# afford-motion/afford-motion

Hardware: AMD Instinct MI355X
Metric: denoising steps/sec (B=32, L=196, N=8192) (higher is better)
Workload: dtype f32

## Files before the change

afford-motion_amd/afm/cmdm.py:

```python
from __future__ import annotations

import ctypes as C
import math
from typing import Dict, List, Optional

import torch
import torch.nn as nn

from . import autograd as AG
from . import ffi, ops
from ._cache import HeldKey
from .base import Model
from .scene import SceneMapEncoder, SceneMapEncoderDecoder
from .text import TextEncoderMixin, lang_feat_dim_type


def compute_repr_dimesion(data_repr: str) -> int:
    table = {"smplx_no_hands": 69, "pos": 66, "pos_rot": 129, "contact_one_joints": 1, "contact_all_joints": 22,
             "contact_cont_joints": 6, "contact_pelvis": 1, "h3d": 263}
    if data_repr not in table:
        raise ValueError(f"Unknown data representation: {data_repr}")
    return table[data_repr]


# ... 148 lines not shown
        self.all_queries = False
        self.no_ln_fold = False
        self.pair_launch = False
        self.fused_layernorm = False
        self._pack = None
        self._cond_cache = None
        self._ws: Dict[tuple, torch.Tensor] = {}

    def _weights(self) -> ffi.CmdmWeights:
        ver = (_param_version(self), self.training)
        if self._pack is not None and self._pack[0] == ver:
            return self._stamp(self._pack[1])
        dev = self.motion_adapter.weight.device
        if dev.type != "cuda":
            raise ffi.AfmError("CMDM parameters are on the CPU; move the model to the MI355X (`model.to('cuda')`)")
        keep: List[torch.Tensor] = []

        def P(t: torch.Tensor) -> int:
            t = ffi.f32c(t.detach())
            keep.append(t)
            return t.data_ptr()

        w = ffi.CmdmWeights()
        layers = self.self_attn_layer.layers
        w.d, w.heads, w.ff, w.n_layers = self.latent_dim, self.num_heads, layers[0].linear1.out_features, len(layers)
        w.motion_dim = self.motion_dim
        w.n_cond = 1 + self.contact_encoder.num_groups
        kpad = -(-self.motion_dim // 16) * 16
        w.motion_adapter_kpad = kpad if (kpad != self.motion_dim and kpad >= 128) else 0
        maw = self.motion_adapter.weight.detach()
        if w.motion_adapter_kpad:
            maw = torch.nn.functional.pad(maw, (0, kpad - self.motion_dim))
        w.motion_adapter_w, w.motion_adapter_b = P(maw), P(self.motion_adapter.bias)
        w.motion_layer_w, w.motion_layer_b = P(self.motion_layer.weight), P(self.motion_layer.bias)
        w.time_table, w.n_timesteps = P(self.timestep_embedder.table()), self.timestep_embedder.pe.shape[0]
        w.pos_table = P(self.positional_encoder.pe[:, 0, :])
        for i, l in enumerate(layers):
            lw = w.layer[i]
            lw.in_proj_w, lw.in_proj_b = P(l.self_attn.in_proj_weight), P(l.self_attn.in_proj_bias)
            lw.out_proj_w, lw.out_proj_b = P(l.self_attn.out_proj.weight), P(l.self_attn.out_proj.bias)
            lw.lin1_w, lw.lin1_b, lw.lin2_w, lw.lin2_b = P(l.linear1.weight), P(l.linear1.bias), P(l.linear2.weight), P(l.linear2.bias)
            lw.norm1_w, lw.norm1_b, lw.norm2_w, lw.norm2_b = P(l.norm1.weight), P(l.norm1.bias), P(l.norm2.weight), P(l.norm2.bias)
        if not self.training:
            import numpy as np

            def fold(lin_w, lin_b, norm):
                wd = lin_w.detach().cpu().numpy().astype(np.float64)
                gam, bet = norm.weight.detach().cpu().numpy().astype(np.float64), norm.bias.detach().cpu().numpy().astype(np.float64)
                wg = wd * gam[None, :]
                up = lambda a: torch.from_numpy(np.ascontiguousarray(a.astype(np.float32))).to(dev)
                return P(up(wg)), P(up(wg.sum(1))), P(up(lin_b.detach().cpu().numpy().astype(np.float64) + wd @ bet))
            for i, l in enumerate(layers):
                lw = w.layer[i]
                lw.lin1_wg, lw.lin1_g, lw.lin1_c = fold(l.linear1.weight, l.linear1.bias, l.norm1)
                if i > 0:
                    lw.in_proj_wg, lw.in_proj_g, lw.in_proj_c = fold(l.self_attn.in_proj_weight, l.self_attn.in_proj_bias, layers[i - 1].norm2)
            w.motion_layer_wg, w.motion_layer_g, w.motion_layer_c = fold(self.motion_layer.weight, self.motion_layer.bias, layers[-1].norm2)
        self._pack = (ver, w, keep)
        return self._stamp(w)

    def _stamp(self, w: ffi.CmdmWeights) -> ffi.CmdmWeights:
        w.gemm_arith, w.gemm_arith_min_n = ops.gemm_arith()
        w.attn_group_waves = int(self.attn_group_waves)
        w.flags = (ffi.CMDM_NO_L0_CACHE if self.no_l0_cache else 0) | (ffi.CMDM_FUSED_LN if self.fused_layernorm else 0) | \
            (ffi.CMDM_NO_LN_FOLD if self.no_ln_fold else 0) | (ffi.CMDM_ALL_QUERIES if self.all_queries else 0) | (ffi.CMDM_NO_RIDERS if self.no_riders else 0) | ((int(self.gemm_tile) & 0xF) << 8) | \
            (ffi.CMDM_PAIR_LAUNCH if self.pair_launch else 0)
        return w

    def _workspace(self, w: ffi.CmdmWeights, B: int, L: int, device) -> torch.Tensor:
        key = (B, L, str(device))
        if key not in self._ws:
            nbytes = ffi.load().afm_cmdm_workspace_bytes(C.byref(w), B, L)
            if nbytes < 0:
# ... 375 lines not shown
```

afford-motion_amd/afm/ffi.py:

```python
from __future__ import annotations

import ctypes as C
import os
from typing import Optional

import torch

_LIB_PATH = os.path.join(os.path.dirname(os.path.abspath(__file__)), "libafm_hip.so")
_lib = None

ACT_NONE, ACT_GELU, ACT_RELU, ACT_SILU = 0, 1, 2, 3
ARITH_DEFAULT, ARITH_F32, ARITH_BF16X1, ARITH_BF16X6, ARITH_BF16X9 = 0, 1, 3, 6, 9
TUNE_NO_DMA, TUNE_TILE_SHIFT = 0x1, 4
CMDM_NO_L0_CACHE, CMDM_FUSED_LN, CMDM_NO_LN_FOLD, CMDM_ALL_QUERIES, CMDM_CLIP_X0, CMDM_NO_RIDERS, CMDM_PAIR_LAUNCH = 0x1, 0x2, 0x4, 0x8, 0x10, 0x20, 0x40
CDM_NO_GEN, CDM_CHAIN_SIDE, CDM_DEC_CHUNKS_SHIFT, CDM_CLIP_X0, CDM_PIPELINE = 0x2, 0x4, 12, 0x8, 0x10
ABI_VERSION = 7
MAX_LAYERS = 16

c_f32p = C.c_void_p
i32, i64, u64 = C.c_int32, C.c_int64, C.c_uint64


class AfmError(RuntimeError):
    pass
# ... 119 lines not shown
                ("per_sample", i64), ("seed", u64), ("sample_index0", i64), ("step", i32)]


class ImputeStepArgs(C.Structure):
    _fields_ = [("x0_c", c_f32p), ("x0_u", c_f32p), ("scale", c_f32p), ("known", c_f32p), ("mask", C.c_void_p), ("x_t", c_f32p),
                ("noise", c_f32p), ("x_next", c_f32p), ("c1", c_f32p), ("c2", c_f32p), ("sigma", c_f32p), ("ddim", C.POINTER(DdimRows)),
                ("clip", i32), ("B", i32), ("per_sample", i64), ("seed", u64), ("sample_index0", i64), ("step", i32)]


CFG_FORCE_MASKED = 0x1

EXPORTS = {
    "afm_version": (C.c_int, []),
    "afm_linear": (C.c_int, [C.POINTER(LinearArgs), C.c_void_p]),
    "afm_linear_pair": (C.c_int, [C.POINTER(LinearArgs), C.POINTER(LinearArgs), C.c_void_p]),
    "afm_mha_fwd": (C.c_int, [c_f32p, C.c_void_p, c_f32p, i32, i32, i32, i32, C.c_void_p]),
    "afm_mha_fwd_grouped": (C.c_int, [c_f32p, C.c_void_p, c_f32p, i32, i32, i32, i32, i32, C.c_void_p]),
    "afm_clamp": (C.c_int, [c_f32p, i64, C.c_float, C.c_float, C.c_void_p]),
    "afm_mha_fwd_rows": (C.c_int, [c_f32p, C.c_void_p, c_f32p, i32, i32, i32, i32, i32, i32, C.c_void_p]),
    "afm_mha_fwd_arith": (C.c_int, [c_f32p, C.c_void_p, c_f32p, i32, i32, i32, i32, i32, i32, i32, C.c_void_p]),
    "afm_mha_cross_fwd": (C.c_int, [c_f32p, c_f32p, C.c_void_p, c_f32p, i32, i32, i32, i32, i32, C.c_void_p]),
    "afm_layernorm": (C.c_int, [c_f32p, c_f32p, c_f32p, c_f32p, i64, i32, C.c_float, C.c_void_p]),
    "afm_layernorm_rows": (C.c_int, [c_f32p, c_f32p, c_f32p, c_f32p, i64, i32, C.c_float, i32, i32, i32, C.c_void_p]),
    "afm_ddpm_step": (C.c_int, [c_f32p, c_f32p, c_f32p, c_f32p, c_f32p, c_f32p, c_f32p, i32, i64, u64, i64, i32, C.c_void_p]),
    "afm_randn": (C.c_int, [c_f32p, i32, i64, u64, i64, i32, C.c_void_p]),
    "afm_ddim_step": (C.c_int, [c_f32p, c_f32p, c_f32p, c_f32p, C.POINTER(DdimRows), i32, i64, u64, i64, i32, C.c_void_p]),
    "afm_ddim_sched_scratch_bytes": (i64, [i32, i32]),
    "afm_cmdm_ddim_loop_range": (C.c_int, [C.POINTER(CmdmWeights), c_f32p, c_f32p, C.c_void_p, c_f32p, C.c_void_p, C.POINTER(DdimRows),
                                           i32, i32, u64, i64, i32, i32, C.c_void_p, C.c_void_p, i64, i32, C.POINTER(C.c_void_p), C.c_void_p]),
    "afm_cdm_ddim_loop_range": (C.c_int, [C.POINTER(CdmWeights), c_f32p, c_f32p, c_f32p, c_f32p, c_f32p, c_f32p, C.c_void_p, C.POINTER(DdimRows),
# ... 179 lines not shown


def require_gpu(*tensors: torch.Tensor) -> None:
    for t in tensors:
        if t is not None and not t.is_cuda:
            raise AfmError("afford-motion_amd runs on the MI355X HIP path only; got a CPU tensor "
                           "(the CPU oracle lives in oracle/ and is test infrastructure)")


def f32c(t: torch.Tensor) -> torch.Tensor:
    if t.dtype != torch.float32:
        t = t.float()
    return t if t.is_contiguous() else t.contiguous()


def profile_enable(on: bool) -> None:
    check(load().afm_profile_enable(1 if on else 0), "afm_profile_enable")


def profile_read():
    buf = (ProfileEntry * 32)()
    n = load().afm_profile_read(buf, 32)
    if n < 0:
        check(n, "afm_profile_read")
    return {buf[i].name.decode(): dict(launches=buf[i].launches, total_ms=buf[i].total_ms, total_work=buf[i].total_work)
            for i in range(n)}


def progress_slices(n_steps: int, progress: bool, slices: int = 50):
    if not progress:
# ... 53 lines not shown
```

afford-motion_amd/csrc/cmdm.hip:

```cpp
#include <memory>

#include "sample_loop.h"

using namespace afm_loop;

extern "C" int afm_linear(const afm_linear_args*, void*);
extern "C" int afm_linear_pair(const afm_linear_args*, const afm_linear_args*, void*);
extern "C" int afm_mha_fwd_grouped(const float*, const uint8_t*, float*, int32_t, int32_t, int32_t, int32_t, int32_t, void*);
extern "C" int afm_mha_fwd_rows(const float*, const uint8_t*, float*, int32_t, int32_t, int32_t, int32_t, int32_t, int32_t, void*);
extern "C" int afm_mha_fwd_arith(const float*, const uint8_t*, float*, int32_t, int32_t, int32_t, int32_t, int32_t, int32_t, int32_t, void*);
extern "C" int afm_layernorm(const float*, const float*, const float*, float*, int64_t, int32_t, float, void*);
extern "C" int afm_layernorm_rows(const float*, const float*, const float*, float*, int64_t, int32_t, float, int32_t, int32_t, int32_t, void*);
extern "C" int afm_randn(float*, int32_t, int64_t, uint64_t, int64_t, int32_t, void*);

namespace {

struct Workspace {
    float *seq0, *y, *x1, *tmp, *qkv, *qkv0, *att, *hid, *noise, *xpad;
    float* x0;
    uint8_t* keymask;
    uint32_t* lncnt;
    float *stat1, *stat2;
    int64_t bytes;
};
// ... 409 lines not shown
        sb = {};
        sub_range(a.B, p->nsub, s, &sb.start, &sb.count);
        off += carve_sub(*c.w, c.cfg ? &p->wu : nullptr, c.L, (char*)a.workspace + off, &sb);
        sb.stream = p->nsub > 1 ? (hipStream_t)a.streams[s] : (hipStream_t)a.stream;
        if (p->branch_streams) sb.branch = (hipStream_t)c.cfg->branch_streams[s];
    }
    if (off > a.workspace_bytes) return AFM_E_WORKSPACE;

    const int T = 1 + c.w->n_cond + c.L;
    p->w = *c.w;
    p->w.flags = a.loop_flags(p->w.flags);
    if (c.cfg || c.mask) p->w.flags = (p->w.flags | AFM_PRIV_DDIM) & ~(AFM_CMDM_PAIR_LAUNCH | AFM_CMDM_FUSED_LN);
    if (p->nsub >= 2 && ((p->w.flags >> AFM_CMDM_WIDE_TILE_SHIFT) & 0xF) == 0) {
        bool big = true;
        for (int s = 0; s < p->nsub; ++s) big = big && (int64_t)p->sb[s].count * T >= 4096;
        if (big) p->w.flags |= 14 << AFM_CMDM_WIDE_TILE_SHIFT;
    }
    if (c.cfg) { const int nc_u = p->wu.n_cond; p->wu = p->w; p->wu.n_cond = nc_u; }
    p->paired = (p->w.flags & AFM_CMDM_PAIR_LAUNCH) && p->nsub == 2 && p->sb[0].count > 0 && p->sb[1].count > 0;
    p->row = (int64_t)c.L * c.w->motion_dim;
    return 0;
}

struct Loop {
    const LoopCall& c;
    LoopPlan p;
    Schedule sched;
};

inline float* sub_x(const Loop& l, const SubBatch& sb) { return l.c.x + (int64_t)sb.start * l.p.row; }

// ... 211 lines not shown
```

afford-motion_amd/csrc/gemm.hip:

```cpp
#include <type_traits>
#include "common.h"
#include "profile.h"
#include "gemm_epilogue.h"

namespace {

constexpr int BK = 32;
constexpr int LDK = 36;

template <int ROWS, bool VEC>
__device__ __forceinline__ void load_tile(const float* const (&rowp)[ROWS / 32], int k, int K, float4 (&reg)[ROWS / 32]) {
#pragma unroll
    for (int i = 0; i < ROWS / 32; ++i) {
        if (VEC) {
            reg[i] = *reinterpret_cast<const float4*>(rowp[i] + min(k, K - 4));
        } else {
            const float* p = rowp[i];
            reg[i] = make_float4(p[min(k, K - 1)], p[min(k + 1, K - 1)], p[min(k + 2, K - 1)], p[min(k + 3, K - 1)]);
        }
    }
}

template <int ROWS>
__device__ __forceinline__ void store_tile(float* __restrict__ lds, int tid, const float4 (&reg)[ROWS / 32], int k, int K) {
// ... 366 lines not shown
    if (lnfold || a.aux_dst) return AFM_E_UNSUPPORTED;
    const bool dma = vec && (a.K % BK) == 0 && !(a.tune & AFM_TUNE_NO_DMA);
    if (!dma) return launch_regs(a, vec, s);
    int tile = (a.tune & AFM_TUNE_TILE_MASK) >> AFM_TUNE_TILE_SHIFT;
    if (tile == 0) {
        const int64_t t64 = (int64_t)((a.M + 63) / 64) * ((a.N + 63) / 64), t3264 = (int64_t)((a.M + 31) / 32) * ((a.N + 63) / 64);
        tile = t64 >= 512 ? 3 : (t3264 >= 512 ? 2 : 1);
    }
    if (a.rowdot_w && tile == 1) tile = 2;
    switch (tile) {
        case 1: return launch_dma<1, 1, 1, 1>(a, AFM_PROF_GEMM32_DMA, s);
        case 2: return launch_dma<1, 2, 1, 1>(a, AFM_PROF_GEMM32x64_DMA, s);
        case 3: return launch_dma<2, 2, 1, 1>(a, AFM_PROF_GEMM64_DMA, s);
        case 4: return launch_dma<2, 2, 1, 2>(a, AFM_PROF_GEMM64x128_DMA, s);
        case 5:
        case 14: return launch_dma<2, 2, 2, 2>(a, AFM_PROF_GEMM128_DMA, s);
        default: return AFM_E_BADARG;
    }
}

int afm_linear_pair_split(const afm_linear_args& a0, const afm_linear_args& a1, int mode, hipStream_t s);
extern "C" int afm_linear_pair(const afm_linear_args* args0, const afm_linear_args* args1, void* stream) {
    if (!args0 || !args1) return AFM_E_BADARG;
    if (args0->M == 0) return afm_linear(args1, stream);
    if (args1->M == 0) return afm_linear(args0, stream);
    if (const int rc = validate_linear(*args0)) return rc;
    if (const int rc = validate_linear(*args1)) return rc;
    const int m0 = afm_linear_split_mode(*args0), m1 = afm_linear_split_mode(*args1);
    if (m0 == 0 || m0 != m1 || args0->K <= 256 || args1->K <= 256) return AFM_E_UNSUPPORTED;
    return afm_linear_pair_split(*args0, *args1, m0, (hipStream_t)stream);
}
// ... 1 lines not shown
```

afford-motion_amd/csrc/gemm_split.hip:

```cpp
#include <type_traits>
#include "common.h"
#include "profile.h"
#include "gemm_epilogue.h"
#include "bf16split.h"

bool afm_linear_rowdot_slab_ok(const afm_linear_args& a);
int afm_linear_rowdot_slab(const afm_linear_args& a, int products, hipStream_t s);

namespace {

constexpr int KSEG = 256;

#ifndef AFM_ABLATE
#define AFM_ABLATE 0
#endif
#ifndef AFM_SPLITK_PIPELINED
#define AFM_SPLITK_PIPELINED 1
#endif

template <int BM, int BN, int BKS, int NPROD, int KG = 1, int RING = 2, int GSEG = 1>
__global__ __launch_bounds__(256 * KG, KG == 1 ? 2 : 1) void gemm_f32_split_bf16(const afm_linear_args p, int nbm, int nbn) {
#define AFM_WG ((int)blockIdx.x)
#define AFM_TIDX threadIdx.x
#define AFM_TIMELINE_SLOT blockIdx.x
// ... 29 lines not shown

template <int BM, int NPROD>
__global__ __launch_bounds__(512, BM == 128 ? 4 : 1) void gemm_f32_split_bf16_wide(const afm_linear_args p, int nbm, int nbn) {
    constexpr int BN = 128, BKS = 16, KG = 1, RING = 2, GSEG = 1;
#define AFM_BODY_WM 4
#define AFM_WG ((int)blockIdx.x)
#define AFM_TIDX threadIdx.x
#define AFM_TIMELINE_SLOT blockIdx.x
#include "gemm_split_body.inc"
#undef AFM_WG
#undef AFM_TIDX
#undef AFM_TIMELINE_SLOT
#undef AFM_BODY_WM
}

inline bool split_offsets_fit_u32(const afm_linear_args& a) {
    const int64_t arow = a.a_grp ? (int64_t)((a.M - 1) / a.a_grp) * a.a_stride + a.a_off + (a.a_grp - 1) + (a.a_skip > 0 ? a.a_skip : 0) : (int64_t)a.M - 1;
    const int64_t amax = (arow * a.lda + a.K) * 4, wmax = ((int64_t)(a.N - 1) * a.ldw + a.K) * 4;
    return a.a_stride >= 0 && a.a_off >= 0 && arow >= 0 && amax < (int64_t(1) << 32) && wmax < (int64_t(1) << 32);
}

template <int BM, int BN, int BKS, int NPROD, int KG = 1, int RING = 2, int GSEG = 1>
int launch_split(const afm_linear_args& a, hipStream_t s);

template <int BM, int NPROD>
int launch_split_wide(const afm_linear_args& a, hipStream_t s) {
    static_assert(BM == 128 || BM == 256, "512-thread tiles: 128 x 128 or 256 x 128");
    constexpr int BN = 128, BKS = 16;
    constexpr int STAGE = 3 * (BM + BN) * (BKS * 2 + 16);
    constexpr int OPER = 2 * STAGE > BM * (BN + 4) * 4 ? 2 * STAGE : BM * (BN + 4) * 4;
    constexpr int LDS_BYTES = OPER + 2 * BM * 2 * 4;
    static_assert(LDS_BYTES <= (BM == 128 ? 80 : 160) * 1024, "LDS of one CU (the 128 x 128 form: two workgroups per CU)");
    if (BM > 128 && a.ln_out) return AFM_E_UNSUPPORTED;
    if (BM == 128 && !split_offsets_fit_u32(a)) return launch_split<128, 128, 16, NPROD, 1, 2, 1>(a, s);
    if (a.aux_dst && a.aux_rows > (int64_t)((a.M + BM - 1) / BM) * ((a.N + BN - 1) / BN)) return AFM_E_UNSUPPORTED;
    static const int attr = []() {
        return (int)hipFuncSetAttribute((const void*)gemm_f32_split_bf16_wide<BM, NPROD>, hipFuncAttributeMaxDynamicSharedMemorySize, LDS_BYTES);
    }();
    if (attr != 0) return attr;
    const int nbm = (a.M + BM - 1) / BM, nbn = (a.N + BN - 1) / BN;
    AfmProf prof(AFM_PROF_GEMM_SPLIT128, 2.0 * a.M * a.N * a.K, s);
    hipLaunchKernelGGL((gemm_f32_split_bf16_wide<BM, NPROD>), dim3(nbm * nbn), dim3(512), LDS_BYTES, s, a, nbm, nbn);
    AFM_CHECK_LAUNCH();
    return 0;
}

struct afm_linear_pair_args {
    afm_linear_args a[2];
    int nbm[2], nbn[2];
    int tiles0, start1;
};
template <int BM, int BN, int BKS, int NPROD>
__global__ __launch_bounds__(256, 2) void gemm_f32_split_bf16_pair(const afm_linear_pair_args pa) {
    constexpr int KG = 1, RING = 2, GSEG = 1;
    const int which = (int)blockIdx.x >= pa.start1 ? 1 : 0;
    const int wg_ = (int)blockIdx.x - (which ? pa.start1 : 0);
    if (!which && wg_ >= pa.tiles0) return;
// ... 86 lines not shown
        if (splittable && (tile == 7 || (tile == 0 && tiles64 <= (nseg == 2 ? 512 : 256)))) {
            if (nseg == 2) return launch_split<64, 64, 16, NPROD, 2>(a, s);
            if (nseg == 3) return launch_split<64, 64, 16, NPROD, 3>(a, s);
            return launch_split<64, 64, 16, NPROD, 4>(a, s);
        }
        if (tile == 7) return AFM_E_UNSUPPORTED;
    }
    if (tile == 9 && (a.K % 64) != 0) return AFM_E_UNSUPPORTED;
    if (tile == 9) return launch_split<64, 64, 16, NPROD, 1, 3>(a, s);
    const int64_t tiles128 = (int64_t)((a.M + 127) / 128) * ((a.N + 127) / 128);
    const int64_t resident = 512, rounds = (tiles128 + resident - 1) / resident;
    const bool full_rounds = tiles128 * 10 >= rounds * resident * 9 && a.K > KSEG;
    if (tile == 12) return launch_split_walk<NPROD>(a, s);
    if (tile == 13) return launch_split_wide<256, NPROD>(a, s);
    if (tile == 14) return launch_split_wide<128, NPROD>(a, s);
    if (tile == 3 || (tile != 5 && !full_rounds)) {
        const int64_t tiles64w = (int64_t)((a.M + 63) / 64) * ((a.N + 63) / 64);
        if (tile != 3 && AFM_WALK_GRID > 0 && tiles64w > AFM_WALK_GRID) return launch_split_walk<NPROD>(a, s);
        return launch_split<64, 64, 16, NPROD>(a, s);
    }
    return launch_split<128, 128, 16, NPROD>(a, s);
}

}

int afm_linear_split_mode(const afm_linear_args& a) {
    int mode, min_n;
    switch (a.arith) {
        case AFM_ARITH_DEFAULT: mode = 6; min_n = 32; break;
        case AFM_ARITH_BF16X9: mode = 9; min_n = a.arith_min_n; break;
// ... 19 lines not shown
```

afford-motion_amd/csrc/gemm_split_body.inc:

```
    static_assert(BKS == 16, "one K16 MFMA step per K-tile");
    static_assert(RING == 2 || RING == 3, "two or three LDS stages");
    static_assert(GSEG == 1 || (GSEG == 2 && KG > 1), "two segments per group: split-K forms only");
    static_assert(RING != 3 || KG == 1 || (GSEG * 256 / BKS) % 4 == 0, "three-stage K loop: K-tiles per group must be a multiple of four");
#ifdef AFM_BODY_WM
    constexpr int WMv = AFM_BODY_WM;
#else
    constexpr int WMv = 2;
#endif
    constexpr int GT = WMv * 2 * 64;
    static_assert(WMv == 2 || KG == 1, "groups of more than 256 threads: one K group only");
    constexpr int TM = BM / (WMv * 32), TN = BN / 64;
    static_assert(KG == 1 || (BM == 64 && BN == 64), "the split-K form exists for 64x64 tiles");
    constexpr int ROWB = BKS * 2 + 16;
    constexpr int ROWS = BM + BN;
    constexpr int PLANE = ROWS * ROWB;
    constexpr int STAGE = 3 * PLANE;
    constexpr int NA = BM * 4 / GT, NW = BN * 4 / GT;
    constexpr int NI = NA + NW;
    constexpr int LDC = BN + 4;
    extern __shared__ __attribute__((aligned(16))) unsigned char lds_raw[];
    const int grp = KG > 1 ? __builtin_amdgcn_readfirstlane((int)(AFM_TIDX >> 8)) : 0;
    unsigned char* lds = lds_raw + grp * (RING * STAGE);
#if defined(AFM_TIMELINE) && defined(AFM_DESYNC_TICKS)
    if ((AFM_WG >> 8) & 1) {
        const unsigned long long td = __builtin_amdgcn_s_memrealtime();
        while (__builtin_amdgcn_s_memrealtime() - td < AFM_DESYNC_TICKS) __builtin_amdgcn_s_sleep(20);
    }
#endif
#ifdef AFM_TIMELINE
    const unsigned long long tl_t0 = __builtin_amdgcn_s_memrealtime(), tl_c0 = afm_cycles();
#endif

    const int nblk = nbm * nbn;
    int bid = AFM_WG;
    {
        const int xcd = bid & 7, idx = bid >> 3, q = nblk >> 3, r = nblk & 7;
        bid = (xcd < r ? xcd * (q + 1) : r * (q + 1) + (xcd - r) * q) + idx;
    }
    const int bm = bid / nbn, bn = bid % nbn;
    const int tid = AFM_TIDX & (GT - 1), lane = tid & 63, wave = tid >> 6;
    const int wm = wave >> 1, wn = wave & 1;
    const int r32 = lane & 31, hh = lane >> 5;

    constexpr bool SOFF = GT == 512 && BM == 128;
    const RowMap amap{p.a_grp, p.a_stride, p.a_off, p.a_skip_after, p.a_skip};
    const float* src[NI];
    uint32_t soff[NI];
    int dst[NI];
#pragma unroll
    for (int i = 0; i < NI; ++i) {
        const int it = tid + GT * (i < NA ? i : i - NA), q = it & 3, v = it >> 2, row = (v & ~7) + ((v & 3) << 1) + ((v >> 2) & 1);
        const int64_t eoff = (i < NA ? amap(min(bm * BM + row, p.M - 1)) * p.lda : (int64_t)min(bn * BN + row, p.N - 1) * p.ldw) + q * 4 + grp * (GSEG * KSEG);
        src[i] = (i < NA ? p.A : p.W) + eoff;
        soff[i] = (uint32_t)eoff * 4u;
        dst[i] = ((i < NA ? 0 : BM) + row) * ROWB + q * 8;
    }

    f32x16 acc[TM][TN];
#pragma unroll
// ... 20 lines not shown
        if ((AFM_ABLATE & 1) && kt >= 2) {
#pragma unroll
            for (int i = 0; i < NI; ++i) asm volatile("" : "+v"(g[S][i]));
            return;
        }
#pragma unroll
        for (int i = 0; i < NI; ++i) {
            if ((AFM_ABLATE & 32) && i >= NA && kt >= 2) { asm volatile("" : "+v"(g[S][i])); continue; }
            if ((AFM_ABLATE & 64) && i < NA && kt >= 2) { asm volatile("" : "+v"(g[S][i])); continue; }
            if constexpr (SOFF) g[S][i] = *reinterpret_cast<const f32x4*>(reinterpret_cast<const unsigned char*>(i < NA ? p.A : p.W) + (soff[i] + (uint32_t)k * 4u));
            else g[S][i] = *reinterpret_cast<const f32x4*>(src[i] + k);
        }
    };
    using Set0 = std::integral_constant<int, 0>;
    using Set1 = std::integral_constant<int, 1>;
    load(Set0{}, 0);
    load(Set1{}, 1);
    constexpr int ROWST_OFF = KG * RING * STAGE > BM * LDC * 4 ? KG * RING * STAGE : BM * LDC * 4;
    float* rowst = reinterpret_cast<float*>(lds_raw + ROWST_OFF);
    gemm_rowstats<BM>(p, rowst, bm);
    auto split_set = [&](auto SETC, int stage) {
        constexpr int S = decltype(SETC)::value;
#pragma unroll
        for (int i = 0; i < NI; ++i) {
            unsigned char* d = lds + stage * STAGE + dst[i];
            uint32_t a1, a2, a3, b1, b2, b3;
            split2(g[S][i][0], g[S][i][1], a1, a2, a3);
            split2(g[S][i][2], g[S][i][3], b1, b2, b3);
            *reinterpret_cast<u32x2*>(d) = u32x2{a1, b1};
            *reinterpret_cast<u32x2*>(d + PLANE) = u32x2{a2, b2};
            *reinterpret_cast<u32x2*>(d + 2 * PLANE) = u32x2{a3, b3};
        }
    };
    using Set2 = std::integral_constant<int, 2>;
    using Set3 = std::integral_constant<int, 3>;
    if constexpr (RING == 3) {
        load(Set2{}, 2);
        load(Set3{}, 3);
        split_set(Set0{}, 0);
        load(Set0{}, 4);
        split_set(Set1{}, 1);
    } else {
        split_set(Set0{}, 0);
        if constexpr (SOFF) {
#pragma unroll
            for (int i = 0; i < NI; ++i) g[0][i] = g[1][i];
        }
    }
    __syncthreads();
#ifdef AFM_TIMELINE
    const unsigned long long tl_pro = __builtin_amdgcn_s_memrealtime();
#endif

    const int a_off = (wm * (BM / WMv) + r32) * ROWB + hh * 16;
    const int w_off = (BM + wn * (BN / 2) + r32) * ROWB + hh * 16;
    constexpr int NMFMA = NPROD * TM * TN;
    constexpr int NPIECE = NI * 2 * 3;

    uint4 af[TM][3], bf[TN][3];
    auto body = [&](auto CURC, int kt) {
        constexpr int cur = decltype(CURC)::value;
        constexpr int RS = SOFF ? 0 : cur ^ 1;
        if constexpr (!SOFF) load(CURC, kt + 2);
        const unsigned char* base = lds + cur * STAGE;
        unsigned char* wbase = lds + (cur ^ 1) * STAGE;
        float r0[NI * 2], r1[NI * 2];
        uint32_t sp[NI * 2][3];
        int piece = 0, m = 0;
        auto do_piece = [&](int t) {
            const int u = t / 3, lvl = t % 3, i = u / 2, c = u % 2;
            if ((AFM_ABLATE & 32) && i >= NA && kt >= 1) return;
            if ((AFM_ABLATE & 64) && i < NA && kt >= 1) return;
            if (lvl == 0) {
                r0[u] = g[RS][i][2 * c];
                r1[u] = g[RS][i][2 * c + 1];
            }
            const uint32_t pk = (AFM_ABLATE & 2) ? __float_as_uint(lvl == 1 ? r1[u] : r0[u]) : cvt_pk_bf16(r0[u], r1[u]);
            sp[u][lvl] = pk;
            if (lvl < 2) {
// ... 6 lines not shown
                if (AFM_ABLATE & 4) {
#pragma unroll
                    for (int pl = 0; pl < 3; ++pl) asm volatile("" :: "v"(sp[2 * i][pl]), "v"(sp[2 * i + 1][pl]), "v"(d));
                } else {
#pragma unroll
                    for (int pl = 0; pl < 3; ++pl) *reinterpret_cast<u32x2*>(d + pl * PLANE) = u32x2{sp[2 * i][pl], sp[2 * i + 1][pl]};
                }
            }
        };
        if (!(AFM_ABLATE & 8) || kt == 0)
#pragma unroll
        for (int pl = 0; pl < 3; ++pl) {
#pragma unroll
            for (int i = 0; i < TM; ++i) af[i][pl] = *reinterpret_cast<const uint4*>(base + pl * PLANE + a_off + i * 32 * ROWB);
#pragma unroll
            for (int j = 0; j < TN; ++j) bf[j][pl] = *reinterpret_cast<const uint4*>(base + pl * PLANE + w_off + j * 32 * ROWB);
        }
        __builtin_amdgcn_sched_barrier(0);
#pragma unroll
        for (int q = 9 - NPROD; q < 9; ++q)
#pragma unroll
            for (int tm = 0; tm < TM; ++tm)
#pragma unroll
                for (int tn = 0; tn < TN; ++tn) {
                    if (AFM_ABLATE & 16) asm volatile("" : "+v"(acc[tm][tn][q]) : "v"(af[tm][AFM_PA[q]].x), "v"(af[tm][AFM_PA[q]].w), "v"(bf[tn][AFM_PB[q]].x), "v"(bf[tn][AFM_PB[q]].w));
                    else acc[tm][tn] = mfma_bf16(af[tm][AFM_PA[q]], bf[tn][AFM_PB[q]], acc[tm][tn]);
                    ++m;
#pragma unroll
                    for (int t = 0; t < NPIECE; ++t)
                        if (t >= piece && t < (m * NPIECE) / NMFMA) do_piece(t);
                    if constexpr (SOFF) {
#pragma unroll
                        for (int i = 0; i < NI; ++i)
                            if (piece < (i + 1) * 6 && (m * NPIECE) / NMFMA >= (i + 1) * 6) load_item(Set0{}, i, kt + 2);
                    }
                    piece = (m * NPIECE) / NMFMA;
                    __builtin_amdgcn_sched_barrier(0);
                }
        if ((KG == 1 || GSEG > 1) && ((kt + 1) % SEGT) == 0 && kt + 1 < nk) {
#pragma unroll
            for (int tm = 0; tm < TM; ++tm)
#pragma unroll
                for (int tn = 0; tn < TN; ++tn)
#pragma unroll
                    for (int r = 0; r < 16; ++r) {
                        tot[tm][tn][r] = have_tot ? tot[tm][tn][r] + acc[tm][tn][r] : acc[tm][tn][r];
                        acc[tm][tn][r] = 0.f;
                    }
            have_tot = true;
        }
        __syncthreads();
// ... 175 lines not shown
```

include/afm_hip.h:

```cpp
#ifndef AFM_HIP_H
#define AFM_HIP_H

#include <stdint.h>

#ifdef __cplusplus
extern "C" {
#endif

#define AFM_ABI_VERSION 7

#define AFM_E_BADARG   (-1)
#define AFM_E_WORKSPACE (-2)
#define AFM_E_UNSUPPORTED (-3)

#define AFM_ACT_NONE 0
#define AFM_ACT_GELU 1
#define AFM_ACT_RELU 2
#define AFM_ACT_SILU 3

int afm_version(void);

typedef struct {
    const float* A; int64_t lda;
    const float* W; int64_t ldw;
// ... 26 lines not shown
} afm_linear_args;

#define AFM_ARITH_DEFAULT 0
#define AFM_ARITH_F32     1
#define AFM_ARITH_BF16X1  3
#define AFM_ARITH_BF16X6  6
#define AFM_ARITH_BF16X9  9

#define AFM_TUNE_NO_DMA      0x1
#define AFM_TUNE_TILE_SHIFT  4
#define AFM_TUNE_TILE_MASK   0xF0

int afm_linear(const afm_linear_args* args, void* stream);
int afm_linear_pair(const afm_linear_args* args0, const afm_linear_args* args1, void* stream);


int afm_mha_fwd(const float* qkv, const uint8_t* key_mask, float* out,
                int32_t B, int32_t T, int32_t H, int32_t dh, void* stream);
int afm_mha_fwd_grouped(const float* qkv, const uint8_t* key_mask, float* out,
                        int32_t B, int32_t T, int32_t H, int32_t dh, int32_t group_waves, void* stream);
int afm_mha_fwd_rows(const float* qkv, const uint8_t* key_mask, float* out,
                     int32_t B, int32_t T, int32_t H, int32_t dh, int32_t q_first, int32_t group_waves, void* stream);
int afm_mha_fwd_arith(const float* qkv, const uint8_t* key_mask, float* out,
                      int32_t B, int32_t T, int32_t H, int32_t dh, int32_t q_first, int32_t group_waves, int32_t arith, void* stream);

int afm_mha_cross_fwd(const float* q, const float* kv, const uint8_t* key_mask, float* out,
                      int32_t B, int32_t Tq, int32_t Tk, int32_t H, int32_t dh, void* stream);

int afm_layernorm(const float* x, const float* gamma, const float* beta, float* y,
                  int64_t rows, int32_t dim, float eps, void* stream);
// ... 369 lines not shown
```

Measured before the change: 632.7.

## Pre-split weights into bf16 plane images and DMA them directly into LDS

Adds a one-time per-weight-pack build of pre-split bf16x3 plane images in the LDS tile layout, with a swizzle, for the wide GEMM weights. Registers them in a pointer-keyed table. A new wide-tile mode (15) launches a split GEMM variant that copies these images straight into LDS with global_load_lds, instead of loading f32 weights and splitting them into bf16 planes every tile. This removes the repeated per-tile weight conversion work and register traffic. In exchange it adds image memory, a lookup under a mutex on every launch, and a more complex pipeline schedule.

```diff
diff --git a/afford-motion_amd/afm/cmdm.py b/afford-motion_amd/afm/cmdm.py
--- a/afford-motion_amd/afm/cmdm.py
+++ b/afford-motion_amd/afm/cmdm.py
@@ -186,7 +186,17 @@
         dev = self.motion_adapter.weight.device
         if dev.type != "cuda":
             raise ffi.AfmError("CMDM parameters are on the CPU; move the model to the MI355X (`model.to('cuda')`)")
+        if self._pack is not None and len(self._pack) > 3 and self._pack[3] is not None:
+            self._pack[3].close()
+        self._pack = None
         keep: List[torch.Tensor] = []
+        wide: List[torch.Tensor] = []
+
+        def PW(t: torch.Tensor) -> int:
+            t = ffi.f32c(t.detach())
+            keep.append(t)
+            wide.append(t)
+            return t.data_ptr()
 
         def P(t: torch.Tensor) -> int:
             t = ffi.f32c(t.detach())
@@ -203,15 +213,15 @@
         maw = self.motion_adapter.weight.detach()
         if w.motion_adapter_kpad:
             maw = torch.nn.functional.pad(maw, (0, kpad - self.motion_dim))
-        w.motion_adapter_w, w.motion_adapter_b = P(maw), P(self.motion_adapter.bias)
+        w.motion_adapter_w, w.motion_adapter_b = (PW if w.motion_adapter_kpad else P)(maw), P(self.motion_adapter.bias)
         w.motion_layer_w, w.motion_layer_b = P(self.motion_layer.weight), P(self.motion_layer.bias)
         w.time_table, w.n_timesteps = P(self.timestep_embedder.table()), self.timestep_embedder.pe.shape[0]
         w.pos_table = P(self.positional_encoder.pe[:, 0, :])
         for i, l in enumerate(layers):
             lw = w.layer[i]
-            lw.in_proj_w, lw.in_proj_b = P(l.self_attn.in_proj_weight), P(l.self_attn.in_proj_bias)
-            lw.out_proj_w, lw.out_proj_b = P(l.self_attn.out_proj.weight), P(l.self_attn.out_proj.bias)
-            lw.lin1_w, lw.lin1_b, lw.lin2_w, lw.lin2_b = P(l.linear1.weight), P(l.linear1.bias), P(l.linear2.weight), P(l.linear2.bias)
+            lw.in_proj_w, lw.in_proj_b = (PW if i == 0 else P)(l.self_attn.in_proj_weight), P(l.self_attn.in_proj_bias)
+            lw.out_proj_w, lw.out_proj_b = PW(l.self_attn.out_proj.weight), P(l.self_attn.out_proj.bias)
+            lw.lin1_w, lw.lin1_b, lw.lin2_w, lw.lin2_b = P(l.linear1.weight), P(l.linear1.bias), PW(l.linear2.weight), P(l.linear2.bias)
             lw.norm1_w, lw.norm1_b, lw.norm2_w, lw.norm2_b = P(l.norm1.weight), P(l.norm1.bias), P(l.norm2.weight), P(l.norm2.bias)
         if not self.training:
             import numpy as np
@@ -221,14 +231,19 @@
                 gam, bet = norm.weight.detach().cpu().numpy().astype(np.float64), norm.bias.detach().cpu().numpy().astype(np.float64)
                 wg = wd * gam[None, :]
                 up = lambda a: torch.from_numpy(np.ascontiguousarray(a.astype(np.float32))).to(dev)
-                return P(up(wg)), P(up(wg.sum(1))), P(up(lin_b.detach().cpu().numpy().astype(np.float64) + wd @ bet))
+                return (PW if wide_w else P)(up(wg)), P(up(wg.sum(1))), P(up(lin_b.detach().cpu().numpy().astype(np.float64) + wd @ bet))
+            wide_w = True
             for i, l in enumerate(layers):
                 lw = w.layer[i]
                 lw.lin1_wg, lw.lin1_g, lw.lin1_c = fold(l.linear1.weight, l.linear1.bias, l.norm1)
                 if i > 0:
                     lw.in_proj_wg, lw.in_proj_g, lw.in_proj_c = fold(l.self_attn.in_proj_weight, l.self_attn.in_proj_bias, layers[i - 1].norm2)
+            wide_w = False
             w.motion_layer_wg, w.motion_layer_g, w.motion_layer_c = fold(self.motion_layer.weight, self.motion_layer.bias, layers[-1].norm2)
-        self._pack = (ver, w, keep)
+        planes = None
+        if not self.training:
+            planes = ffi.WeightPlanes([t for t in wide if t.shape[1] % 16 == 0 and t.data_ptr() % 16 == 0])
+        self._pack = (ver, w, keep, planes)
         return self._stamp(w)
 
     def _stamp(self, w: ffi.CmdmWeights) -> ffi.CmdmWeights:
diff --git a/afford-motion_amd/afm/ffi.py b/afford-motion_amd/afm/ffi.py
--- a/afford-motion_amd/afm/ffi.py
+++ b/afford-motion_amd/afm/ffi.py
@@ -157,6 +157,11 @@
     "afm_version": (C.c_int, []),
     "afm_linear": (C.c_int, [C.POINTER(LinearArgs), C.c_void_p]),
     "afm_linear_pair": (C.c_int, [C.POINTER(LinearArgs), C.POINTER(LinearArgs), C.c_void_p]),
+    "afm_weight_planes_bytes": (i64, [i32, i32]),
+    "afm_weight_planes_build": (C.c_int, [c_f32p, i32, i32, i64, C.c_void_p, C.c_void_p]),
+    "afm_weight_planes_register": (C.c_int, [c_f32p, i32, i32, i64, C.c_void_p]),
+    "afm_weight_planes_unregister": (C.c_int, [c_f32p]),
+    "afm_weight_planes_stats": (C.c_int, [C.POINTER(i64), C.POINTER(i64)]),
     "afm_mha_fwd": (C.c_int, [c_f32p, C.c_void_p, c_f32p, i32, i32, i32, i32, C.c_void_p]),
     "afm_mha_fwd_grouped": (C.c_int, [c_f32p, C.c_void_p, c_f32p, i32, i32, i32, i32, i32, C.c_void_p]),
     "afm_clamp": (C.c_int, [c_f32p, i64, C.c_float, C.c_float, C.c_void_p]),
@@ -366,6 +371,50 @@
     return t if t.is_contiguous() else t.contiguous()
 
 
+def weight_planes_image(w: torch.Tensor) -> torch.Tensor:
+    require_gpu(w)
+    assert w.dtype == torch.float32 and w.dim() == 2 and w.stride(1) == 1, "a row-major float32 matrix"
+    lib = load()
+    N, K = w.shape
+    nbytes = int(lib.afm_weight_planes_bytes(N, K))
+    if nbytes < 0:
+        check(nbytes, "afm_weight_planes_bytes")
+    image = torch.empty(nbytes, dtype=torch.uint8, device=w.device)
+    check(lib.afm_weight_planes_build(w.data_ptr(), N, K, w.stride(0), image.data_ptr(), stream_of(w)), "afm_weight_planes_build")
+    return image
+
+
+class WeightPlanes:
+
+    def __init__(self, weights):
+        import weakref
+        self._held = []
+        ptrs = []
+        lib = load()
+        for w in weights:
+            image = weight_planes_image(w)
+            check(lib.afm_weight_planes_register(w.data_ptr(), w.shape[0], w.shape[1], w.stride(0), image.data_ptr()), "afm_weight_planes_register")
+            self._held.append((w, image))
+            ptrs.append(w.data_ptr())
+        self._fin = weakref.finalize(self, WeightPlanes._release, ptrs, self._held)
+
+    @staticmethod
+    def _release(ptrs, held):
+        lib = load()
+        for p in ptrs:
+            lib.afm_weight_planes_unregister(p)
+        del held[:]
+
+    def close(self) -> None:
+        self._fin()
+
+
+def weight_planes_stats():
+    h, m = i64(0), i64(0)
+    check(load().afm_weight_planes_stats(C.byref(h), C.byref(m)), "afm_weight_planes_stats")
+    return int(h.value), int(m.value)
+
+
 def profile_enable(on: bool) -> None:
     check(load().afm_profile_enable(1 if on else 0), "afm_profile_enable")
 
diff --git a/afford-motion_amd/csrc/cmdm.hip b/afford-motion_amd/csrc/cmdm.hip
--- a/afford-motion_amd/csrc/cmdm.hip
+++ b/afford-motion_amd/csrc/cmdm.hip
@@ -447,7 +447,7 @@
     if (p->nsub >= 2 && ((p->w.flags >> AFM_CMDM_WIDE_TILE_SHIFT) & 0xF) == 0) {
         bool big = true;
         for (int s = 0; s < p->nsub; ++s) big = big && (int64_t)p->sb[s].count * T >= 4096;
-        if (big) p->w.flags |= 14 << AFM_CMDM_WIDE_TILE_SHIFT;
+        if (big) p->w.flags |= 15 << AFM_CMDM_WIDE_TILE_SHIFT;
     }
     if (c.cfg) { const int nc_u = p->wu.n_cond; p->wu = p->w; p->wu.n_cond = nc_u; }
     p->paired = (p->w.flags & AFM_CMDM_PAIR_LAUNCH) && p->nsub == 2 && p->sb[0].count > 0 && p->sb[1].count > 0;
diff --git a/afford-motion_amd/csrc/gemm.hip b/afford-motion_amd/csrc/gemm.hip
--- a/afford-motion_amd/csrc/gemm.hip
+++ b/afford-motion_amd/csrc/gemm.hip
@@ -404,7 +404,8 @@
         case 3: return launch_dma<2, 2, 1, 1>(a, AFM_PROF_GEMM64_DMA, s);
         case 4: return launch_dma<2, 2, 1, 2>(a, AFM_PROF_GEMM64x128_DMA, s);
         case 5:
-        case 14: return launch_dma<2, 2, 2, 2>(a, AFM_PROF_GEMM128_DMA, s);
+        case 14:
+        case 15: return launch_dma<2, 2, 2, 2>(a, AFM_PROF_GEMM128_DMA, s);
         default: return AFM_E_BADARG;
     }
 }
diff --git a/afford-motion_amd/csrc/gemm_split.hip b/afford-motion_amd/csrc/gemm_split.hip
--- a/afford-motion_amd/csrc/gemm_split.hip
+++ b/afford-motion_amd/csrc/gemm_split.hip
@@ -6,6 +6,7 @@
 
 bool afm_linear_rowdot_slab_ok(const afm_linear_args& a);
 int afm_linear_rowdot_slab(const afm_linear_args& a, int products, hipStream_t s);
+const void* afm_weight_planes_lookup(const float* W, int N, int K, int64_t ldw);
 
 namespace {
 
@@ -67,6 +68,22 @@
 #undef AFM_BODY_WM
 }
 
+template <int NPROD>
+__global__ __launch_bounds__(512, 4) void gemm_f32_split_bf16_wplanes(const afm_linear_args p, int nbm, int nbn, const unsigned char* __restrict__ wimg) {
+    constexpr int BM = 128, BN = 128, BKS = 16, KG = 1, RING = 2, GSEG = 1;
+#define AFM_BODY_WM 4
+#define AFM_BODY_WPLANES 1
+#define AFM_WG ((int)blockIdx.x)
+#define AFM_TIDX threadIdx.x
+#define AFM_TIMELINE_SLOT blockIdx.x
+#include "gemm_split_body.inc"
+#undef AFM_WG
+#undef AFM_TIDX
+#undef AFM_TIMELINE_SLOT
+#undef AFM_BODY_WPLANES
+#undef AFM_BODY_WM
+}
+
 inline bool split_offsets_fit_u32(const afm_linear_args& a) {
     const int64_t arow = a.a_grp ? (int64_t)((a.M - 1) / a.a_grp) * a.a_stride + a.a_off + (a.a_grp - 1) + (a.a_skip > 0 ? a.a_skip : 0) : (int64_t)a.M - 1;
     const int64_t amax = (arow * a.lda + a.K) * 4, wmax = ((int64_t)(a.N - 1) * a.ldw + a.K) * 4;
@@ -94,6 +111,27 @@
     const int nbm = (a.M + BM - 1) / BM, nbn = (a.N + BN - 1) / BN;
     AfmProf prof(AFM_PROF_GEMM_SPLIT128, 2.0 * a.M * a.N * a.K, s);
     hipLaunchKernelGGL((gemm_f32_split_bf16_wide<BM, NPROD>), dim3(nbm * nbn), dim3(512), LDS_BYTES, s, a, nbm, nbn);
+    AFM_CHECK_LAUNCH();
+    return 0;
+}
+
+template <int NPROD>
+int launch_split_wplanes(const afm_linear_args& a, hipStream_t s) {
+    constexpr int BM = 128, BN = 128, BKS = 16;
+    constexpr int OPER = 2 * 3 * BM * (BKS * 2 + 16) + 2 * 3 * BN * BKS * 2;
+    constexpr int STAGED = BM * (BN + 4) * 4;
+    constexpr int LDS_BYTES = (OPER > STAGED ? OPER : STAGED) + 2 * BM * 2 * 4;
+    static_assert(LDS_BYTES <= 80 * 1024, "two workgroups per CU");
+    const unsigned char* img = split_offsets_fit_u32(a) ? (const unsigned char*)afm_weight_planes_lookup(a.W, a.N, a.K, a.ldw) : nullptr;
+    if (!img) return launch_split_wide<128, NPROD>(a, s);
+    if (a.aux_dst && a.aux_rows > (int64_t)((a.M + BM - 1) / BM) * ((a.N + BN - 1) / BN)) return AFM_E_UNSUPPORTED;
+    static const int attr = []() {
+        return (int)hipFuncSetAttribute((const void*)gemm_f32_split_bf16_wplanes<NPROD>, hipFuncAttributeMaxDynamicSharedMemorySize, LDS_BYTES);
+    }();
+    if (attr != 0) return attr;
+    const int nbm = (a.M + BM - 1) / BM, nbn = (a.N + BN - 1) / BN;
+    AfmProf prof(AFM_PROF_GEMM_SPLIT128, 2.0 * a.M * a.N * a.K, s);
+    hipLaunchKernelGGL((gemm_f32_split_bf16_wplanes<NPROD>), dim3(nbm * nbn), dim3(512), LDS_BYTES, s, a, nbm, nbn, img);
     AFM_CHECK_LAUNCH();
     return 0;
 }
@@ -210,6 +248,10 @@
     if (tile == 12) return launch_split_walk<NPROD>(a, s);
     if (tile == 13) return launch_split_wide<256, NPROD>(a, s);
     if (tile == 14) return launch_split_wide<128, NPROD>(a, s);
+    if (tile == 15) {
+        if constexpr (NPROD == 1) return launch_split_wide<128, NPROD>(a, s);
+        else return launch_split_wplanes<NPROD>(a, s);
+    }
     if (tile == 3 || (tile != 5 && !full_rounds)) {
         const int64_t tiles64w = (int64_t)((a.M + 63) / 64) * ((a.N + 63) / 64);
         if (tile != 3 && AFM_WALK_GRID > 0 && tiles64w > AFM_WALK_GRID) return launch_split_walk<NPROD>(a, s);
diff --git a/afford-motion_amd/csrc/gemm_split_body.inc b/afford-motion_amd/csrc/gemm_split_body.inc
--- a/afford-motion_amd/csrc/gemm_split_body.inc
+++ b/afford-motion_amd/csrc/gemm_split_body.inc
@@ -7,15 +7,22 @@
 #else
     constexpr int WMv = 2;
 #endif
+#ifdef AFM_BODY_WPLANES
+    constexpr bool WPL = true;
+    static_assert(WMv == 4 && BM == 128 && BN == 128 && KG == 1 && RING == 2, "W planes: the 512-thread 128 x 128 tile");
+#else
+    constexpr bool WPL = false;
+#endif
     constexpr int GT = WMv * 2 * 64;
     static_assert(WMv == 2 || KG == 1, "groups of more than 256 threads: one K group only");
     constexpr int TM = BM / (WMv * 32), TN = BN / 64;
     static_assert(KG == 1 || (BM == 64 && BN == 64), "the split-K form exists for 64x64 tiles");
     constexpr int ROWB = BKS * 2 + 16;
-    constexpr int ROWS = BM + BN;
+    constexpr int ROWS = WPL ? BM : BM + BN;
     constexpr int PLANE = ROWS * ROWB;
     constexpr int STAGE = 3 * PLANE;
-    constexpr int NA = BM * 4 / GT, NW = BN * 4 / GT;
+    constexpr int NA = BM * 4 / GT, NW = WPL ? 0 : BN * 4 / GT;
+    [[maybe_unused]] constexpr int WROWB = BKS * 2, WPLANE = BN * WROWB, WSTAGE = 3 * WPLANE, WOFF = RING * STAGE, WPIECES = WSTAGE / 1024;
     constexpr int NI = NA + NW;
     constexpr int LDC = BN + 4;
     extern __shared__ __attribute__((aligned(16))) unsigned char lds_raw[];
@@ -43,6 +50,10 @@
     const int r32 = lane & 31, hh = lane >> 5;
 
     constexpr bool SOFF = GT == 512 && BM == 128;
+#ifndef AFM_WPL_TWO_SETS
+#define AFM_WPL_TWO_SETS 0
+#endif
+    constexpr bool ONESET = SOFF && !(WPL && AFM_WPL_TWO_SETS);
     const RowMap amap{p.a_grp, p.a_stride, p.a_off, p.a_skip_after, p.a_skip};
     const float* src[NI];
     uint32_t soff[NI];
@@ -93,9 +104,23 @@
     };
     using Set0 = std::integral_constant<int, 0>;
     using Set1 = std::integral_constant<int, 1>;
+    [[maybe_unused]] auto w_dma = [&](int kt, int stage) {
+#ifdef AFM_BODY_WPLANES
+        static_assert(WPIECES == 12, "eight waves: four move two pieces, four move one");
+        const int wv = __builtin_amdgcn_readfirstlane(wave);
+        const int pc = wv < 4 ? 2 * wv : 4 + wv;
+        const unsigned char* gs = wimg + ((size_t)bn * nk + kt) * WSTAGE + pc * 1024 + lane * 16;
+        unsigned char* ld = lds + WOFF + stage * WSTAGE + pc * 1024;
+        __builtin_amdgcn_global_load_lds((const __attribute__((address_space(1))) void*)gs, (__attribute__((address_space(3))) void*)ld, 16, 0, 0);
+        if (wv < 4)
+            __builtin_amdgcn_global_load_lds((const __attribute__((address_space(1))) void*)gs, (__attribute__((address_space(3))) void*)ld, 16, 1024, 0);
+#endif
+    };
+    if constexpr (WPL) w_dma(0, 0);
     load(Set0{}, 0);
     load(Set1{}, 1);
-    constexpr int ROWST_OFF = KG * RING * STAGE > BM * LDC * 4 ? KG * RING * STAGE : BM * LDC * 4;
+    constexpr int OPER = KG * RING * STAGE + (WPL ? 2 * WSTAGE : 0);
+    constexpr int ROWST_OFF = OPER > BM * LDC * 4 ? OPER : BM * LDC * 4;
     float* rowst = reinterpret_cast<float*>(lds_raw + ROWST_OFF);
     gemm_rowstats<BM>(p, rowst, bm);
     auto split_set = [&](auto SETC, int stage) {
@@ -121,7 +146,7 @@
         split_set(Set1{}, 1);
     } else {
         split_set(Set0{}, 0);
-        if constexpr (SOFF) {
+        if constexpr (ONESET) {
 #pragma unroll
             for (int i = 0; i < NI; ++i) g[0][i] = g[1][i];
         }
@@ -132,16 +157,18 @@
 #endif
 
     const int a_off = (wm * (BM / WMv) + r32) * ROWB + hh * 16;
-    const int w_off = (BM + wn * (BN / 2) + r32) * ROWB + hh * 16;
+    const int w_off = WPL ? WOFF + (wn * (BN / 2) + r32) * WROWB + ((hh ^ ((r32 >> 4) & 1)) * 16) : (BM + wn * (BN / 2) + r32) * ROWB + hh * 16;
+    constexpr int W_ST = WPL ? WSTAGE : STAGE, W_PL = WPL ? WPLANE : PLANE, W_RB = WPL ? WROWB : ROWB;
     constexpr int NMFMA = NPROD * TM * TN;
     constexpr int NPIECE = NI * 2 * 3;
 
     uint4 af[TM][3], bf[TN][3];
     auto body = [&](auto CURC, int kt) {
         constexpr int cur = decltype(CURC)::value;
-        constexpr int RS = SOFF ? 0 : cur ^ 1;
-        if constexpr (!SOFF) load(CURC, kt + 2);
+        constexpr int RS = ONESET ? 0 : cur ^ 1;
+        if constexpr (!ONESET) load(CURC, kt + 2);
         const unsigned char* base = lds + cur * STAGE;
+        const unsigned char* basew = lds + cur * W_ST;
         unsigned char* wbase = lds + (cur ^ 1) * STAGE;
         float r0[NI * 2], r1[NI * 2];
         uint32_t sp[NI * 2][3];
@@ -178,7 +205,7 @@
 #pragma unroll
             for (int i = 0; i < TM; ++i) af[i][pl] = *reinterpret_cast<const uint4*>(base + pl * PLANE + a_off + i * 32 * ROWB);
 #pragma unroll
-            for (int j = 0; j < TN; ++j) bf[j][pl] = *reinterpret_cast<const uint4*>(base + pl * PLANE + w_off + j * 32 * ROWB);
+            for (int j = 0; j < TN; ++j) bf[j][pl] = *reinterpret_cast<const uint4*>(basew + pl * W_PL + w_off + j * 32 * W_RB);
         }
         __builtin_amdgcn_sched_barrier(0);
 #pragma unroll
@@ -190,15 +217,17 @@
                     if (AFM_ABLATE & 16) asm volatile("" : "+v"(acc[tm][tn][q]) : "v"(af[tm][AFM_PA[q]].x), "v"(af[tm][AFM_PA[q]].w), "v"(bf[tn][AFM_PB[q]].x), "v"(bf[tn][AFM_PB[q]].w));
                     else acc[tm][tn] = mfma_bf16(af[tm][AFM_PA[q]], bf[tn][AFM_PB[q]], acc[tm][tn]);
                     ++m;
+                    if (WPL && m == 1 && kt + 1 < nk) w_dma(kt + 1, cur ^ 1);
+                    const int want = WPL ? (2 * m * NPIECE / NMFMA < NPIECE ? 2 * m * NPIECE / NMFMA : NPIECE) : (m * NPIECE) / NMFMA;
 #pragma unroll
                     for (int t = 0; t < NPIECE; ++t)
-                        if (t >= piece && t < (m * NPIECE) / NMFMA) do_piece(t);
-                    if constexpr (SOFF) {
+                        if (t >= piece && t < want) do_piece(t);
+                    if constexpr (ONESET) {
 #pragma unroll
                         for (int i = 0; i < NI; ++i)
-                            if (piece < (i + 1) * 6 && (m * NPIECE) / NMFMA >= (i + 1) * 6) load_item(Set0{}, i, kt + 2);
+                            if (piece < (i + 1) * 6 && want >= (i + 1) * 6) load_item(Set0{}, i, kt + 2);
                     }
-                    piece = (m * NPIECE) / NMFMA;
+                    piece = want;
                     __builtin_amdgcn_sched_barrier(0);
                 }
         if ((KG == 1 || GSEG > 1) && ((kt + 1) % SEGT) == 0 && kt + 1 < nk) {
diff --git a/afford-motion_amd/csrc/weight_planes.hip b/afford-motion_amd/csrc/weight_planes.hip
--- /dev/null
+++ b/afford-motion_amd/csrc/weight_planes.hip
@@ -0,0 +1,86 @@
+#include <mutex>
+#include <vector>
+#include "common.h"
+#include "bf16split.h"
+
+namespace {
+
+constexpr int BN = 128, BK = 16, BLOB = 3 * BN * BK * 2;
+
+__global__ __launch_bounds__(256) void weight_planes_kernel(const float* __restrict__ W, int N, int K, int64_t ldw, unsigned char* __restrict__ image, int64_t items) {
+    const int64_t it = (int64_t)blockIdx.x * 256 + threadIdx.x;
+    if (it >= items) return;
+    const int kh = K / 8;
+    const int64_t n = it / kh;
+    const int h8 = (int)(it % kh), kt = h8 >> 1, h = h8 & 1;
+    const int bn = (int)(n / BN), r = (int)(n % BN);
+    u32x4 t[3] = {u32x4{0, 0, 0, 0}, u32x4{0, 0, 0, 0}, u32x4{0, 0, 0, 0}};
+    if (n < N) {
+        const float* src = W + n * ldw + h8 * 8;
+        const f32x4 lo = *reinterpret_cast<const f32x4*>(src), hi = *reinterpret_cast<const f32x4*>(src + 4);
+        const float v[8] = {lo[0], lo[1], lo[2], lo[3], hi[0], hi[1], hi[2], hi[3]};
+#pragma unroll
+        for (int c = 0; c < 4; ++c) {
+            uint32_t p1, p2, p3;
+            split2(v[2 * c], v[2 * c + 1], p1, p2, p3);
+            t[0][c] = p1; t[1][c] = p2; t[2][c] = p3;
+        }
+    }
+    unsigned char* blob = image + ((int64_t)bn * (K / BK) + kt) * BLOB;
+    const int off = r * (BK * 2) + ((h ^ ((r >> 4) & 1)) * 16);
+#pragma unroll
+    for (int pl = 0; pl < 3; ++pl) *reinterpret_cast<u32x4*>(blob + pl * (BN * BK * 2) + off) = t[pl];
+}
+
+struct Entry { const float* W; int N, K; int64_t ldw; const void* image; };
+std::mutex g_mu;
+std::vector<Entry> g_tab;
+int64_t g_hits = 0, g_misses = 0;
+
+bool shape_ok(int N, int K, int64_t ldw) { return N > 0 && K > 0 && K % BK == 0 && ldw >= K && ldw % 4 == 0; }
+
+}
+
+const void* afm_weight_planes_lookup(const float* W, int N, int K, int64_t ldw) {
+    std::lock_guard<std::mutex> lk(g_mu);
+    for (const Entry& e : g_tab)
+        if (e.W == W && e.N == N && e.K == K && e.ldw == ldw) { ++g_hits; return e.image; }
+    ++g_misses;
+    return nullptr;
+}
+
+extern "C" int64_t afm_weight_planes_bytes(int N, int K) {
+    if (N <= 0 || K <= 0 || K % BK != 0) return AFM_E_BADARG;
+    return (int64_t)((N + BN - 1) / BN) * (K / BK) * BLOB;
+}
+
+extern "C" int afm_weight_planes_build(const float* W, int N, int K, int64_t ldw, void* image, void* stream) {
+    if (!W || !image || !shape_ok(N, K, ldw) || ((uintptr_t)W & 15) || ((uintptr_t)image & 15)) return AFM_E_BADARG;
+    const int64_t items = (int64_t)((N + BN - 1) / BN) * BN * (K / 8);
+    hipLaunchKernelGGL(weight_planes_kernel, dim3((unsigned)((items + 255) / 256)), dim3(256), 0, (hipStream_t)stream, W, N, K, ldw, (unsigned char*)image, items);
+    AFM_CHECK_LAUNCH();
+    return 0;
+}
+
+extern "C" int afm_weight_planes_register(const float* W, int N, int K, int64_t ldw, const void* image) {
+    if (!W || !image || !shape_ok(N, K, ldw)) return AFM_E_BADARG;
+    std::lock_guard<std::mutex> lk(g_mu);
+    for (Entry& e : g_tab)
+        if (e.W == W && e.N == N && e.K == K && e.ldw == ldw) { e.image = image; return 0; }
+    g_tab.push_back(Entry{W, N, K, ldw, image});
+    return 0;
+}
+
+extern "C" int afm_weight_planes_unregister(const float* W) {
+    std::lock_guard<std::mutex> lk(g_mu);
+    for (size_t i = g_tab.size(); i-- > 0;)
+        if (g_tab[i].W == W) g_tab.erase(g_tab.begin() + i);
+    return 0;
+}
+
+extern "C" int afm_weight_planes_stats(int64_t* hits, int64_t* misses) {
+    std::lock_guard<std::mutex> lk(g_mu);
+    if (hits) *hits = g_hits;
+    if (misses) *misses = g_misses;
+    return 0;
+}
diff --git a/include/afm_hip.h b/include/afm_hip.h
--- a/include/afm_hip.h
+++ b/include/afm_hip.h
@@ -64,6 +64,12 @@
 int afm_linear(const afm_linear_args* args, void* stream);
 int afm_linear_pair(const afm_linear_args* args0, const afm_linear_args* args1, void* stream);
 
+int64_t afm_weight_planes_bytes(int N, int K);
+int afm_weight_planes_build(const float* W, int N, int K, int64_t ldw, void* image, void* stream);
+int afm_weight_planes_register(const float* W, int N, int K, int64_t ldw, const void* image);
+int afm_weight_planes_unregister(const float* W);
+int afm_weight_planes_stats(int64_t* hits, int64_t* misses);
+
 
 int afm_mha_fwd(const float* qkv, const uint8_t* key_mask, float* out,
                 int32_t B, int32_t T, int32_t H, int32_t dh, void* stream);
```

New measurement: 615.2. 0.972x the previous value.
